# gunrock/graphblast

Hardware: NVIDIA H100
Metric: MTEPS (higher is better)
Workload: dtype f32

## Files before the change

graphblast_b200/csrc/graphblas/backend/cuda/kernels/bfs_fused.cuh:

```cuda
#ifndef GRAPHBLAS_BACKEND_CUDA_KERNELS_BFS_FUSED_CUH_
#define GRAPHBLAS_BACKEND_CUDA_KERNELS_BFS_FUSED_CUH_

#include <cooperative_groups.h>

#include "graphblas/backend/cuda/kernels/common.cuh"

namespace graphblas {
namespace backend {

#ifndef GB_BFS_NT
#define GB_BFS_NT     512
#endif
#ifndef GB_BFS_MINB
#define GB_BFS_MINB   2
#endif
#ifndef GB_BFS_PUSH_NT
#define GB_BFS_PUSH_NT   768
#endif
#ifndef GB_BFS_PUSH_MINB
#define GB_BFS_PUSH_MINB 2
#endif
#ifndef GB_BFS_BATCH
#define GB_BFS_BATCH  4
#endif
#ifndef GB_BFS_WALK_STEP
#define GB_BFS_WALK_STEP 4
#endif
#ifndef GB_BFS_WALK_WARP
#define GB_BFS_WALK_WARP 32
#endif
#ifndef GB_BFS_WALK_INLINE
#define GB_BFS_WALK_INLINE 64
#endif
#define GB_BFS_HEAVY  2048
#define GB_BFS_HEAVY_CAP 4096
#define GB_BFS_CHUNK  1024

struct BfsFusedArgs {
  const Index* push_ptr;   const Index* push_ind;
  const Index* pull_ptr;   const Index* pull_ind;
  const Index* pull_probe;
  const unsigned int* pull_empty;
  const unsigned int* push_empty;
  int   trace;
  unsigned long long* prof_bytes;
  Index n;
  Index source;
  int   max_levels;
  float switchpoint;
  int   mode;
  float*        levels;
  unsigned char* level8;
  unsigned int* visited[2];
  unsigned int* frontier;
  unsigned int* next;
  unsigned long long* counters;
  Index*        heavy;
  Index*        walk;
  int*          walk_count;
  Index*        walk_chunks;
};

#define GB_BFS_TIMED_LEVELS 16

enum BfsCell {
  GB_BFS_CELL_FOUND = 0,
  GB_BFS_CELL_HEAVY = GB_BFS_CELL_FOUND + 3,
  GB_BFS_CELL_LEVELS = GB_BFS_CELL_HEAVY + 3,
  GB_BFS_CELL_INSPECTED,
  GB_BFS_CELL_PULL_LEVELS,
  GB_BFS_CELL_PUSHED_VERTICES,
  GB_BFS_CELL_PUSHED_EDGES,
  GB_BFS_CELL_FOUND_PUSHING,
  GB_BFS_CELL_LEVEL_CLOCK,
  GB_BFS_CELL_START_CLOCK = GB_BFS_CELL_LEVEL_CLOCK + GB_BFS_TIMED_LEVELS,
  GB_BFS_CELL_END_PASS_CLOCK,
  GB_BFS_CELL_LAST_LEVEL_CLOCK,
  GB_BFS_CELL_WALK_CLAIM = 35,
  GB_BFS_CELL_LISTED = GB_BFS_CELL_WALK_CLAIM + 3,
  GB_BFS_CELL_SCAN_CLOCK = 44,
  GB_BFS_CELL_WALKED = GB_BFS_CELL_SCAN_CLOCK + GB_BFS_TIMED_LEVELS,
  GB_BFS_CELL_LISTED_CHUNKS = GB_BFS_CELL_WALKED + GB_BFS_TIMED_LEVELS,
  GB_BFS_NCOUNTERS = 128
};
static_assert(GB_BFS_CELL_LISTED_CHUNKS + GB_BFS_TIMED_LEVELS <= GB_BFS_NCOUNTERS,
              "the per-level cells of the last timed level are past the counters");

__device__ __forceinline__ unsigned long long* bfsLevelCell(unsigned long long* cells,
                                                            int first, int level) {
  return cells + first + level % 3;
}
__device__ __forceinline__ void bfsZeroNextCell(unsigned long long* cells, int first,
                                                int level) {
  cells[first + (level + 1) % 3] = 0ull;
}

__device__ __forceinline__ unsigned long long bfsClockNs() {
  unsigned long long t;
  asm volatile("mov.u64 %0, %globaltimer;" : "=l"(t));
  return t;
}

template <typename V>
__device__ __forceinline__ bool bfsClaim(unsigned int* visited, V vtx) {
  const unsigned int bit = 1u << (vtx & 31);
  unsigned int* word = visited + (vtx >> 5);
  if (*reinterpret_cast<volatile unsigned int*>(word) & bit) return false;
  return (atomicOr(word, bit) & bit) == 0;
}

__device__ __forceinline__ void bfsSetLevel(const BfsFusedArgs& a, Index row, int lv) {
  if (lv < 255) {
    a.level8[row] = static_cast<unsigned char>(lv);
  } else {
    a.level8[row] = 255;
    a.levels[row] = static_cast<float>(lv);
  }
}

__device__ __forceinline__ Index bfsClaimChunk(unsigned long long* cell, int lane) {
  unsigned long long c = 0ull;
  if (lane == 0) c = atomicAdd(cell, 1ull);
  return static_cast<Index>(__shfl_sync(GB_FULL_MASK, c, 0));
}

__device__ __forceinline__ unsigned int* bfsVis(const BfsFusedArgs& a, int vsel) {
  return vsel ? a.visited[1] : a.visited[0];
}
__device__ __forceinline__ unsigned int* bfsVisOther(const BfsFusedArgs& a, int vsel) {
  return vsel ? a.visited[0] : a.visited[1];
}
__device__ __forceinline__ unsigned int* bfsF(const BfsFusedArgs& a, int fsel) {
  return fsel ? a.next : a.frontier;
}
__device__ __forceinline__ unsigned int* bfsN(const BfsFusedArgs& a, int fsel) {
  return fsel ? a.frontier : a.next;
}

__device__ __forceinline__ unsigned int bfsIsolated(const BfsFusedArgs& a, Index w) {
  return a.pull_empty[w] & (a.push_empty != NULL ? a.push_empty[w] : 0xffffffffu);
}

__device__ __forceinline__ bool bfsWalkRows(const BfsFusedArgs& a, int vsel, Index row,
                                            bool active, int lane, int& inspected) {
  Index k = 0, end = 0;
  if (active) {
    k = __ldg(a.pull_ptr + row);
    end = __ldg(a.pull_ptr + row + 1);
  }
  const Index stop = (end - k > GB_BFS_WALK_WARP + GB_BFS_WALK_STEP)
                     ? k + GB_BFS_WALK_STEP : end;
  bool found = false;
  while (k < stop && !found) {
    Index col[GB_BFS_WALK_STEP];
    unsigned int wv[GB_BFS_WALK_STEP];
#pragma unroll
    for (int u = 0; u < GB_BFS_WALK_STEP; ++u)
      col[u] = (k + u < stop) ? __ldg(a.pull_ind + k + u) : static_cast<Index>(-1);
#pragma unroll
    for (int u = 0; u < GB_BFS_WALK_STEP; ++u)
      wv[u] = (col[u] >= 0) ? bfsVis(a, vsel)[col[u] >> 5] : 0u;
#pragma unroll
    for (int u = 0; u < GB_BFS_WALK_STEP; ++u) {
      if (found || col[u] < 0) continue;
      ++inspected;
      found = (wv[u] >> (col[u] & 31)) & 1u;
    }
    k += GB_BFS_WALK_STEP;
  }
  unsigned int longs = __ballot_sync(GB_FULL_MASK, !found && k < end);
  while (longs != 0u) {
    const int src = __ffs(longs) - 1;
    longs &= longs - 1u;
    const Index lend = __shfl_sync(GB_FULL_MASK, end, src);
    bool hit = false;
    for (Index lk = __shfl_sync(GB_FULL_MASK, k, src); lk < lend && !hit; lk += 32) {
      bool v = false;
      if (lk + lane < lend) {
        const Index col = __ldg(a.pull_ind + lk + lane);
        v = (bfsVis(a, vsel)[col >> 5] >> (col & 31)) & 1u;
      }
      const unsigned int b = __ballot_sync(GB_FULL_MASK, v);
      hit = (b != 0u);
      if (lane == 0)
        inspected += hit ? __ffs(b) : (lend - lk < 32 ? lend - lk : 32);
    }
    if (lane == src) found = hit;
  }
  return found;
}

template <int NT, int MINB, bool PULL>
__global__ void __launch_bounds__(NT, MINB)
bfsFusedKernel(BfsFusedArgs a) {
  namespace cg = cooperative_groups;
  cg::grid_group grid = cg::this_grid();
  __shared__ int s_red[NT/32];
  __shared__ unsigned int s_found[PULL ? NT/32 : 1][PULL ? 32 : 1];

  const Index n = a.n;
  const Index nwords = (n + 31) >> 5;
  const int lane = threadIdx.x & 31;
  const Index gtid = blockIdx.x*NT + threadIdx.x;
  const Index gthreads = gridDim.x*NT;
  const Index gwarp = gtid >> 5;
  const Index gwarps = gthreads >> 5;
  const Index nchunks = (nwords + 31) >> 5;

  if (gtid == 0) a.counters[GB_BFS_CELL_START_CLOCK] = bfsClockNs();
  if (gtid == 0) a.level8[a.source] = 1;
  for (Index w = gtid; w < nwords; w += gthreads) {
    const unsigned int seed = (w == (a.source >> 5)) ? (1u << (a.source & 31)) : 0u;
    a.visited[0][w] = seed | bfsIsolated(a, w);
    a.visited[1][w] = 0u; a.frontier[w] = seed; a.next[w] = 0u;
  }
  if (gtid <= GB_BFS_CELL_FOUND_PUSHING) a.counters[gtid] = 0ull;
  if (gtid >= GB_BFS_CELL_WALK_CLAIM && gtid < GB_BFS_CELL_LISTED + 3) a.counters[gtid] = 0ull;
  if (gtid >= GB_BFS_CELL_WALKED && gtid < GB_BFS_CELL_WALKED + GB_BFS_TIMED_LEVELS)
    a.counters[gtid] = 0ull;
  grid.sync();
  if (gtid == 0) a.counters[GB_BFS_CELL_LEVEL_CLOCK] = bfsClockNs() << 1;

  int vsel = 0;
  int fsel = 0;
  unsigned int fcount = 1u;
  bool dense = PULL && (a.mode == 2);
  float prev_ratio = 0.f;
  int inspected = 0;
  int pushed_vertices = 0;
  unsigned int pushed_edges = 0u;
  int pull_levels = 0;
  int level = 1;

  for (; level <= a.max_levels && fcount > 0u; ++level) {
    if (PULL && a.mode == 0) {
      const float ratio = static_cast<float>(fcount)/static_cast<float>(n);
      if (!dense) {
        if (ratio > a.switchpoint && ratio > prev_ratio) dense = true; else prev_ratio = ratio;
      } else {
        if (ratio <= a.switchpoint && ratio < prev_ratio) dense = false; else prev_ratio = ratio;
      }
    }
    unsigned long long* const count_cell = bfsLevelCell(a.counters, GB_BFS_CELL_FOUND, level);
    unsigned long long* const heavy_cell = bfsLevelCell(a.counters, GB_BFS_CELL_HEAVY, level);
    if (gtid == 0) {
      bfsZeroNextCell(a.counters, GB_BFS_CELL_FOUND, level);
      bfsZeroNextCell(a.counters, GB_BFS_CELL_HEAVY, level);
      bfsZeroNextCell(a.counters, GB_BFS_CELL_WALK_CLAIM, level);
      bfsZeroNextCell(a.counters, GB_BFS_CELL_LISTED, level);
    }
    int found_here = 0;

    if (!dense) {
      for (Index w0 = gwarp*32; w0 < nwords; w0 += gwarps*32) {
        const Index mine = w0 + lane;
        unsigned int my_bits = (mine < nwords) ? bfsF(a, fsel)[mine] : 0u;
        if (my_bits != 0u) bfsF(a, fsel)[mine] = 0u;
        unsigned int pending = __ballot_sync(GB_FULL_MASK, my_bits != 0u);
        while (pending != 0u) {
          const int src_lane = __ffs(pending) - 1;
          pending &= pending - 1u;
          unsigned int bits = __shfl_sync(GB_FULL_MASK, my_bits, src_lane);
          const Index w = w0 + src_lane;
          while (bits != 0u) {
            const int b = __ffs(bits) - 1;
            bits &= bits - 1u;
            const Index u = w*32 + b;
            const Index beg = __ldg(a.push_ptr + u);
            const Index deg = __ldg(a.push_ptr + u + 1) - beg;
            if (lane == 0) { ++pushed_vertices; pushed_edges += deg; }
            if (deg > GB_BFS_HEAVY) {
              unsigned long long slot = 0ull;
              if (lane == 0) slot = atomicAdd(heavy_cell, 1ull);
              slot = __shfl_sync(GB_FULL_MASK, slot, 0);
              if (slot < GB_BFS_HEAVY_CAP) {
                if (lane == 0) a.heavy[slot] = u;
                continue;
              }
            }
            for (Index k = lane; k < deg; k += 32) {
              const Index nbr = __ldg(a.push_ind + beg + k);
              if (bfsClaim(bfsVis(a, vsel), nbr)) {
                bfsSetLevel(a, nbr, level + 1);
                atomicOr(bfsN(a, fsel) + (nbr >> 5), 1u << (nbr & 31));
                ++found_here;
              }
            }
          }
        }
      }
      grid.sync();
      const unsigned long long listed =
          *reinterpret_cast<volatile unsigned long long*>(heavy_cell);
      const int nheavy = (listed > GB_BFS_HEAVY_CAP) ? GB_BFS_HEAVY_CAP
                                                     : static_cast<int>(listed);
      if (nheavy > 0) {
        for (int h = 0; h < nheavy; ++h) {
          const Index u = a.heavy[h];
          const Index beg = __ldg(a.push_ptr + u);
          const Index deg = __ldg(a.push_ptr + u + 1) - beg;
          for (Index k = gtid; k < deg; k += gthreads) {
            const Index nbr = __ldg(a.push_ind + beg + k);
            if (bfsClaim(bfsVis(a, vsel), nbr)) {
              bfsSetLevel(a, nbr, level + 1);
              atomicOr(bfsN(a, fsel) + (nbr >> 5), 1u << (nbr & 31));
              ++found_here;
            }
          }
        }
      }
    } else if (PULL) {
      ++pull_levels;
      unsigned long long* const walk_cell =
          bfsLevelCell(a.counters, GB_BFS_CELL_WALK_CLAIM, level);
      unsigned long long* const list_cell = bfsLevelCell(a.counters, GB_BFS_CELL_LISTED, level);
      Index c = gwarp;
      unsigned int next_vis = (c < nchunks && c*32 + lane < nwords)
                              ? bfsVis(a, vsel)[c*32 + lane] : 0xffffffffu;
      while (c < nchunks) {
        const Index word = c*32 + lane;
        const unsigned int my_vis = next_vis;
        const Index c_next = c + gwarps;
        next_vis = (c_next < nchunks && c_next*32 + lane < nwords)
                   ? bfsVis(a, vsel)[c_next*32 + lane] : 0xffffffffu;
        Index* const walk = a.walk + c*GB_BFS_CHUNK;
        int nwalk = 0;
        unsigned int my_out = 0u;
        unsigned int open = __ballot_sync(GB_FULL_MASK, my_vis != 0xffffffffu);
        unsigned int my_open = ~my_vis;
        if (word == nwords - 1 && (n & 31) != 0) my_open &= (1u << (n & 31)) - 1u;
        const int nopen = __popc(my_open);
        int first = nopen;
#pragma unroll
        for (int off = 1; off < 32; off <<= 1) {
          const int t = __shfl_up_sync(GB_FULL_MASK, first, off);
          if (lane >= off) first += t;
        }
        const int total = __shfl_sync(GB_FULL_MASK, first, 31);
        first -= nopen;
        const int word_batches = (__popc(open) + GB_BFS_BATCH - 1)/GB_BFS_BATCH;
        const int row_batches = (total + 32*GB_BFS_BATCH - 1)/(32*GB_BFS_BATCH);
        if (2*row_batches < word_batches) {
          open = 0u;
          unsigned int* const found_bits = s_found[threadIdx.x >> 5];
          found_bits[lane] = 0u;
          __syncwarp();
          for (int r0 = 0; r0 < total; r0 += 32*GB_BFS_BATCH) {
            int local[GB_BFS_BATCH];
            Index f[GB_BFS_BATCH];
#pragma unroll
            for (int j = 0; j < GB_BFS_BATCH; ++j) {
              const int r = r0 + 32*j + lane;
              int wl = 0, base = 0;
#pragma unroll
              for (int step = 16; step > 0; step >>= 1) {
                const int fs = __shfl_sync(GB_FULL_MASK, first, wl + step);
                if (fs <= r) { wl += step; base = fs; }
              }
              unsigned int m = __shfl_sync(GB_FULL_MASK, my_open, wl);
              int k = r - base, b = 0;
#pragma unroll
              for (int width = 16; width > 0; width >>= 1) {
                const int lo = __popc(m & ((1u << width) - 1u));
                if (k >= lo) { k -= lo; b += width; m >>= width; }
              }
              local[j] = wl*32 + b;
              f[j] = (r < total) ? ldStream32(a.pull_probe + c*GB_BFS_CHUNK + local[j])
                                 : static_cast<Index>(-1);
            }
            unsigned int pword[GB_BFS_BATCH];
#pragma unroll
            for (int j = 0; j < GB_BFS_BATCH; ++j)
              pword[j] = (f[j] != static_cast<Index>(-1))
                         ? bfsVis(a, vsel)[(f[j] & 0x7fffffff) >> 5] : 0u;
#pragma unroll
            for (int j = 0; j < GB_BFS_BATCH; ++j) {
              if (r0 + 32*j >= total) break;
              const bool found = (pword[j] >> (f[j] & 31)) & 1u;
              inspected += (f[j] != static_cast<Index>(-1)) ? 1 : 0;
              const bool walk_row = f[j] >= 0 && !found;
              const Index row = c*GB_BFS_CHUNK + local[j];
              const unsigned int walkers = __ballot_sync(GB_FULL_MASK, walk_row);
              if (walk_row) walk[nwalk + __popc(walkers & ((1u << lane) - 1u))] = row;
              nwalk += __popc(walkers);
              if (found) {
                atomicOr(found_bits + (local[j] >> 5), 1u << (local[j] & 31));
                bfsSetLevel(a, row, level + 1);
                ++found_here;
              }
            }
          }
          __syncwarp();
          my_out = found_bits[lane];
        }
        while (open != 0u) {
          const unsigned int batch = open;
          Index f[GB_BFS_BATCH];
#pragma unroll
          for (int j = 0; j < GB_BFS_BATCH; ++j) {
            const int wl = __ffs(open) - 1;
            open &= open - 1u;
            f[j] = static_cast<Index>(-1);
            if (wl >= 0) {
              const unsigned int m = __shfl_sync(GB_FULL_MASK, my_vis, wl);
              const Index row = c*GB_BFS_CHUNK + wl*32 + lane;
              if (row < n && !((m >> lane) & 1u)) f[j] = ldStream32(a.pull_probe + row);
            }
          }
          unsigned int pword[GB_BFS_BATCH];
#pragma unroll
          for (int j = 0; j < GB_BFS_BATCH; ++j)
            pword[j] = (f[j] != static_cast<Index>(-1))
                       ? bfsVis(a, vsel)[(f[j] & 0x7fffffff) >> 5] : 0u;
          unsigned int hit = 0u, more = 0u;
#pragma unroll
          for (int j = 0; j < GB_BFS_BATCH; ++j) {
            const bool found = (pword[j] >> (f[j] & 31)) & 1u;
            inspected += (f[j] != static_cast<Index>(-1)) ? 1 : 0;
            hit |= static_cast<unsigned int>(found) << j;
            more |= static_cast<unsigned int>(f[j] >= 0 && !found) << j;
          }
          unsigned int rest = batch;
#pragma unroll
          for (int j = 0; j < GB_BFS_BATCH && rest != 0u; ++j) {
            const int wl = __ffs(rest) - 1;
            rest &= rest - 1u;
            const Index row = c*GB_BFS_CHUNK + wl*32 + lane;
            const bool found = (hit >> j) & 1u, walk_row = (more >> j) & 1u;
            const unsigned int walkers = __ballot_sync(GB_FULL_MASK, walk_row);
            if (walk_row) walk[nwalk + __popc(walkers & ((1u << lane) - 1u))] = row;
            nwalk += __popc(walkers);
            const unsigned int out = __ballot_sync(GB_FULL_MASK, found);
            if (found) { bfsSetLevel(a, row, level + 1); ++found_here; }
            if (lane == wl) my_out = out;
          }
        }
        if (nwalk > 0 && nwalk <= GB_BFS_WALK_INLINE) {
          unsigned int* const found_bits = s_found[threadIdx.x >> 5];
          found_bits[lane] = my_out;
          __syncwarp();
          for (int i0 = 0; i0 < nwalk; i0 += 32) {
            const bool active = i0 + lane < nwalk;
            const Index row = active ? walk[i0 + lane] : 0;
            if (bfsWalkRows(a, vsel, row, active, lane, inspected)) {
              const int local = row & (GB_BFS_CHUNK - 1);
              atomicOr(found_bits + (local >> 5), 1u << (local & 31));
              bfsSetLevel(a, row, level + 1);
              ++found_here;
            }
          }
          __syncwarp();
          my_out = found_bits[lane];
        }
        if (word < nwords) {
          bfsN(a, fsel)[word] = my_out;
          bfsVisOther(a, vsel)[word] = my_vis | my_out;
          bfsF(a, fsel)[word] = 0u;
        }
        if (lane == 0 && nwalk > 0) {
          if (nwalk > GB_BFS_WALK_INLINE) {
            a.walk_count[c] = nwalk;
            a.walk_chunks[atomicAdd(list_cell, 1ull)] = c;
          }
          if (a.trace && level < GB_BFS_TIMED_LEVELS)
            atomicAdd(a.counters + GB_BFS_CELL_WALKED + level,
                      static_cast<unsigned long long>(nwalk));
        }
        c = c_next;
      }
      grid.sync();
      const Index nlisted = static_cast<Index>(
          *reinterpret_cast<volatile unsigned long long*>(list_cell));
      if (gtid == 0 && level < GB_BFS_TIMED_LEVELS) {
        a.counters[GB_BFS_CELL_SCAN_CLOCK + level] = bfsClockNs();
        if (a.trace)
          a.counters[GB_BFS_CELL_LISTED_CHUNKS + level] = static_cast<unsigned long long>(nlisted);
      }
      for (Index i = gwarp; i < nlisted; ) {
        const Index i_next = gwarps + bfsClaimChunk(walk_cell, lane);
        const Index c = a.walk_chunks[i];
        const int nwalk = a.walk_count[c];
        for (int i0 = 0; i0 < nwalk; i0 += 32) {
          const bool active = i0 + lane < nwalk;
          const Index row = active ? a.walk[c*GB_BFS_CHUNK + i0 + lane] : 0;
          if (bfsWalkRows(a, vsel, row, active, lane, inspected)) {
            const unsigned int bit = 1u << (row & 31);
            atomicOr(bfsN(a, fsel) + (row >> 5), bit);
            atomicOr(bfsVisOther(a, vsel) + (row >> 5), bit);
            bfsSetLevel(a, row, level + 1);
            ++found_here;
          }
        }
        i = i_next;
      }
    }
    const int block_found = blockSum<NT>(found_here, s_red);
    if (threadIdx.x == 0 && block_found) {
      atomicAdd(count_cell, static_cast<unsigned long long>(block_found));
      if (!dense)
        atomicAdd(a.counters + GB_BFS_CELL_FOUND_PUSHING,
                  static_cast<unsigned long long>(block_found));
    }
    grid.sync();
    if (gtid == 0 && level < GB_BFS_TIMED_LEVELS)
      a.counters[GB_BFS_CELL_LEVEL_CLOCK + level] = (bfsClockNs() << 1) | (dense ? 1ull : 0ull);
    fcount = static_cast<unsigned int>(
        *reinterpret_cast<volatile unsigned long long*>(count_cell));
    if (dense) vsel ^= 1;
    fsel ^= 1;
  }
  if (gtid == 0) a.counters[GB_BFS_CELL_LAST_LEVEL_CLOCK] = bfsClockNs();
  const unsigned int* const cut_rows = (fcount > 0u) ? bfsF(a, fsel) : NULL;
  const bool lines = (reinterpret_cast<uintptr_t>(a.levels) & 15u) == 0u;
  const Index nblocks = (nwords + 15) >> 4;
  if (PULL) {
    auto load_block = [&](Index blk, unsigned int& reached, unsigned int (&b)[4]) {
      reached = 0u;
#pragma unroll
      for (int j = 0; j < 4; ++j) b[j] = 0u;
      if (blk >= nblocks) return;
      const Index w = blk*16 + (lane & 15);
      if (lane < 16 && w < nwords) {
        reached = bfsVis(a, vsel)[w] & ~bfsIsolated(a, w);
        if (cut_rows != NULL) reached &= ~cut_rows[w];
        if (w == (a.source >> 5)) reached |= 1u << (a.source & 31);
      }
#pragma unroll
      for (int j = 0; j < 4; ++j) {
        const Index row = blk*512 + 128*j + 4*lane;
        if (lines && row + 4 <= n) b[j] = *reinterpret_cast<const unsigned int*>(a.level8 + row);
      }
    };
    unsigned int next_reached, next_b[4];
    load_block(gwarp, next_reached, next_b);
    for (Index blk = gwarp; blk < nblocks; blk += gwarps) {
      const Index r0 = blk*512;
      const unsigned int reached = next_reached;
      unsigned int lb[4];
#pragma unroll
      for (int j = 0; j < 4; ++j) lb[j] = next_b[j];
      load_block(blk + gwarps, next_reached, next_b);
#pragma unroll
      for (int j = 0; j < 4; ++j) {
        const unsigned int bits =
            (__shfl_sync(GB_FULL_MASK, reached, 4*j + (lane >> 3)) >> (4*(lane & 7))) & 0xfu;
        const Index row = r0 + 128*j + 4*lane;
        if (row >= n) continue;
        if (lines && row + 4 <= n) {
          const unsigned int b = lb[j];
          float f[4];
          bool escape = false;
#pragma unroll
          for (int k = 0; k < 4; ++k) {
            const unsigned int byte = (b >> (8*k)) & 0xffu;
            const bool r = (bits >> k) & 1u;
            escape |= r && byte == 255u;
            f[k] = r ? static_cast<float>(byte) : 0.f;
          }
          if (!escape) {
            __stcs(reinterpret_cast<float4*>(a.levels + row), make_float4(f[0], f[1], f[2], f[3]));
            continue;
          }
        }
        for (int k = 0; k < 4 && row + k < n; ++k) {
          if (!((bits >> k) & 1u)) {
            a.levels[row + k] = 0.f;
          } else {
            const unsigned int byte = a.level8[row + k];
            if (byte != 255u) a.levels[row + k] = static_cast<float>(byte);
          }
        }
      }
    }
  } else {
    for (Index blk = gwarp; blk < nblocks; blk += gwarps) {
      const Index r0 = blk*512;
      const Index w = blk*16 + (lane & 15);
      unsigned int reached = 0u;
      if (lane < 16 && w < nwords) {
        reached = bfsVis(a, vsel)[w] & ~bfsIsolated(a, w);
        if (cut_rows != NULL) reached &= ~cut_rows[w];
        if (w == (a.source >> 5)) reached |= 1u << (a.source & 31);
      }
#pragma unroll
      for (int j = 0; j < 4; ++j) {
        const unsigned int bits =
            (__shfl_sync(GB_FULL_MASK, reached, 4*j + (lane >> 3)) >> (4*(lane & 7))) & 0xfu;
        const Index row = r0 + 128*j + 4*lane;
        if (row >= n) continue;
        if (lines && row + 4 <= n) {
          const unsigned int b = *reinterpret_cast<const unsigned int*>(a.level8 + row);
          float f[4];
          bool escape = false;
#pragma unroll
          for (int k = 0; k < 4; ++k) {
            const unsigned int byte = (b >> (8*k)) & 0xffu;
            const bool r = (bits >> k) & 1u;
            escape |= r && byte == 255u;
            f[k] = r ? static_cast<float>(byte) : 0.f;
          }
          if (!escape) {
            __stcs(reinterpret_cast<float4*>(a.levels + row), make_float4(f[0], f[1], f[2], f[3]));
            continue;
          }
        }
        for (int k = 0; k < 4 && row + k < n; ++k) {
          if (!((bits >> k) & 1u)) {
            a.levels[row + k] = 0.f;
          } else {
            const unsigned int byte = a.level8[row + k];
            if (byte != 255u) a.levels[row + k] = static_cast<float>(byte);
          }
        }
      }
    }
  }
  if (a.trace) {
    grid.sync();
    if (gtid == 0) a.counters[GB_BFS_CELL_END_PASS_CLOCK] = bfsClockNs();
  }
  const int block_insp = blockSum<NT>(inspected, s_red);
  const int block_pv = blockSum<NT>(pushed_vertices, s_red);
  if (threadIdx.x == 0) {
    if (block_insp)
      atomicAdd(a.counters + GB_BFS_CELL_INSPECTED, static_cast<unsigned long long>(block_insp));
    if (block_pv)
      atomicAdd(a.counters + GB_BFS_CELL_PUSHED_VERTICES,
                static_cast<unsigned long long>(block_pv));
  }
  if (pushed_edges)
    atomicAdd(a.counters + GB_BFS_CELL_PUSHED_EDGES,
              static_cast<unsigned long long>(pushed_edges));
  if (gtid == 0) {
    a.counters[GB_BFS_CELL_LEVELS] = static_cast<unsigned long long>(level - 1);
    a.counters[GB_BFS_CELL_PULL_LEVELS] = static_cast<unsigned long long>(pull_levels);
  }
  if (a.prof_bytes != NULL) {
    if (pushed_edges) atomicAdd(a.prof_bytes, 8ull*pushed_edges);
    if (threadIdx.x == 0) {
      unsigned long long bytes = 4ull*static_cast<unsigned long long>(block_insp) +
                                 12ull*static_cast<unsigned long long>(block_pv);
      if (blockIdx.x == 0)
        bytes += static_cast<unsigned long long>(pull_levels)*
                     (12ull*static_cast<unsigned long long>(n) + 4ull) +
                 8ull*(*reinterpret_cast<volatile unsigned long long*>(
                           a.counters + GB_BFS_CELL_FOUND_PUSHING));
      if (bytes) atomicAdd(a.prof_bytes, bytes);
    }
  }
}

}
}

#endif
```

graphblast_b200/csrc/graphblas/backend/cuda/bfs_fused.hpp:

```cpp
#ifndef GRAPHBLAS_BACKEND_CUDA_BFS_FUSED_HPP_
#define GRAPHBLAS_BACKEND_CUDA_BFS_FUSED_HPP_

#include "graphblas/backend/cuda/kernels/bfs_fused.cuh"

namespace graphblas {
namespace backend {

inline bool bfsFusedApplies(Descriptor* desc) {
  Desc_value mask_mode, outp, inp0, inp1;
  if (desc->get(GrB_MASK, &mask_mode) != GrB_SUCCESS) return false;
  desc->get(GrB_OUTP, &outp); desc->get(GrB_INP0, &inp0); desc->get(GrB_INP1, &inp1);
  return desc->struconly() && desc->opreuse() && desc->earlyexit() && desc->fusedmask() &&
         mask_mode == GrB_DEFAULT && outp == GrB_DEFAULT && inp0 == GrB_DEFAULT &&
         inp1 == GrB_DEFAULT && !desc->debug() && desc->timing_ != 1;
}

inline bool bfsTrace() {
  static const bool on = getEnv("GB200_BFS_TRACE", 0) != 0;
  return on;
}

struct BfsScratchLayout {
  size_t visited[2], frontier, next, counters, heavy, walk, walk_count, walk_chunks,
         level8, bytes;
};

inline BfsScratchLayout bfsScratchLayout(Index n) {
  const size_t nwords = (static_cast<size_t>(n) + 31)/32;
  const size_t nchunks = (nwords + 31)/32;
  BfsScratchLayout l;
  size_t at = 0;
  auto place = [&at](size_t bytes) {
    const size_t off = at;
    at += (bytes + 255)/256*256;
    return off;
  };
  l.visited[0]  = place(nwords*sizeof(unsigned int));
  l.visited[1]  = place(nwords*sizeof(unsigned int));
  l.frontier    = place(nwords*sizeof(unsigned int));
  l.next        = place(nwords*sizeof(unsigned int));
  l.counters    = place(GB_BFS_NCOUNTERS*sizeof(unsigned long long));
  l.heavy       = place(GB_BFS_HEAVY_CAP*sizeof(Index));
  l.walk        = place(nchunks*GB_BFS_CHUNK*sizeof(Index));
  l.walk_count  = place(nchunks*sizeof(int));
  l.walk_chunks = place(nchunks*sizeof(Index));
  l.level8      = place(static_cast<size_t>(n));
  l.bytes = at;
  return l;
}

inline void bfsFusedStats(Descriptor* desc, Index n, unsigned long long out[6]) {
  static_assert(GB_BFS_CELL_FOUND_PUSHING == GB_BFS_CELL_LEVELS + 5,
                "the six result cells are not consecutive");
  for (int i = 0; i < 6; ++i) out[i] = 0ull;
  const BfsScratchLayout l = bfsScratchLayout(n);
  const size_t cells = l.counters + GB_BFS_CELL_LEVELS*sizeof(unsigned long long);
  if (desc->scratchSize(GB_SCRATCH_BFS) < cells + 6*sizeof(unsigned long long)) return;
  unsigned char* base = reinterpret_cast<unsigned char*>(desc->scratch(GB_SCRATCH_BFS, 0));
  CUDA_CALL(cudaMemcpyAsync(out, base + cells, 6*sizeof(unsigned long long),
      cudaMemcpyDeviceToHost, gbStream()));
  runtime().sync();
}

template <typename a>
Info bfsFused(Vector<float>* v, const Matrix<a>* A, Index s, Descriptor* desc, int* depth) {
  SparseMatrix<a>* S = const_cast<SparseMatrix<a>*>(&A->sparse_);
  const Index n = S->nrows_;
  if (n != S->ncols_) return GrB_DIMENSION_MISMATCH;
  if (S->d_csrRowPtr_ == NULL || S->d_cscColPtr_ == NULL) return GrB_UNINITIALIZED_OBJECT;
  cudaStream_t stream = gbStream();
  CHECK(v->setStorage(GrB_DENSE));
  CHECK(v->dense_.allocateGpu());

  const int fw = 1;
  const Index* probe = pullMaxDegreeNeighbours(S, fw, S->d_cscColPtr_, S->d_cscRowInd_, n);

  const BfsScratchLayout l = bfsScratchLayout(n);
  unsigned char* base =
      reinterpret_cast<unsigned char*>(desc->scratch(GB_SCRATCH_BFS, l.bytes));
  BfsFusedArgs args;
  args.push_ptr = S->d_csrRowPtr_;  args.push_ind = S->d_csrColInd_;
  args.pull_ptr = S->d_cscColPtr_;  args.pull_ind = S->d_cscRowInd_;
  args.pull_probe = probe;
  args.pull_empty = pullEmptyRowBits(probe, n);
  args.push_empty = S->sameStructure() ? NULL : pullEmptyRowBits(
      pullFirstNeighbours(S, 0, S->d_csrRowPtr_, S->d_csrColInd_, n), n);
  args.n = n;
  args.source = s;
  args.max_levels = desc->max_niter_;
  args.switchpoint = desc->switchpoint();
  Desc_value mode;
  CHECK(desc->get(GrB_MXVMODE, &mode));
  args.mode = (mode == GrB_PUSHONLY) ? 1 : (mode == GrB_PULLONLY ? 2 : 0);
  args.levels = v->dense_.d_val_;
  args.visited[0]  = reinterpret_cast<unsigned int*>(base + l.visited[0]);
  args.visited[1]  = reinterpret_cast<unsigned int*>(base + l.visited[1]);
  args.frontier    = reinterpret_cast<unsigned int*>(base + l.frontier);
  args.next        = reinterpret_cast<unsigned int*>(base + l.next);
  args.counters    = reinterpret_cast<unsigned long long*>(base + l.counters);
  args.heavy       = reinterpret_cast<Index*>(base + l.heavy);
  args.walk        = reinterpret_cast<Index*>(base + l.walk);
  args.walk_count  = reinterpret_cast<int*>(base + l.walk_count);
  args.walk_chunks = reinterpret_cast<Index*>(base + l.walk_chunks);
  args.level8      = base + l.level8;

  args.trace = bfsTrace();
  args.prof_bytes = NULL;
  if (profiler().enabled) {
    profiler().ensureCells();
    args.prof_bytes = profiler().d_cells + GB_PROF_PULL_BOOL;
  }

  const bool push_only = (args.mode == 1);
  void (*kernel)(BfsFusedArgs) =
      push_only ? bfsFusedKernel<GB_BFS_PUSH_NT, GB_BFS_PUSH_MINB, false>
                : bfsFusedKernel<GB_BFS_NT, GB_BFS_MINB, true>;
  const int nt = push_only ? GB_BFS_PUSH_NT : GB_BFS_NT;
  const int grid = push_only
      ? cooperativeGrid<bfsFusedKernel<GB_BFS_PUSH_NT, GB_BFS_PUSH_MINB, false>,
                        GB_BFS_PUSH_NT>()
      : cooperativeGrid<bfsFusedKernel<GB_BFS_NT, GB_BFS_MINB, true>, GB_BFS_NT>();
  if (grid < 1) return GrB_PANIC;
  void* params[] = { &args };
  profiler().begin(GB_PROF_PULL_BOOL, stream);
  CUDA_CALL(cudaLaunchCooperativeKernel(reinterpret_cast<void*>(kernel),
      dim3(grid), dim3(nt), params, 0, stream));
  GB_KERNEL_CHECK();
  profiler().end(GB_PROF_PULL_BOOL, stream, 0.0);
  v->dense_.touched();
  if (args.trace) {
    unsigned long long cells[GB_BFS_NCOUNTERS];
    CUDA_CALL(cudaMemcpyAsync(cells, args.counters, sizeof(cells), cudaMemcpyDeviceToHost,
        stream));
    runtime().sync();
    const unsigned long long* const clock = cells + GB_BFS_CELL_LEVEL_CLOCK;
    const int levels = static_cast<int>(
        cells[GB_BFS_CELL_LEVELS] < GB_BFS_TIMED_LEVELS - 1 ? cells[GB_BFS_CELL_LEVELS]
                                                            : GB_BFS_TIMED_LEVELS - 1);
    fprintf(stderr, "bfs trace: set-up %.1fus",
            1e-3*static_cast<double>((clock[0] >> 1) - cells[GB_BFS_CELL_START_CLOCK]));
    for (int l = 1; l <= levels; ++l) {
      const unsigned long long start = clock[l - 1] >> 1, end = clock[l] >> 1;
      const unsigned long long scan = cells[GB_BFS_CELL_SCAN_CLOCK + l];
      if (clock[l] & 1ull)
        fprintf(stderr, " L%d pull %.1fus (scan %.1f walk %.1f, %llu walked, %llu listed)",
                l, 1e-3*static_cast<double>(end - start),
                1e-3*static_cast<double>(scan - start),
                1e-3*static_cast<double>(end - scan), cells[GB_BFS_CELL_WALKED + l],
                cells[GB_BFS_CELL_LISTED_CHUNKS + l]);
      else
        fprintf(stderr, " L%d push %.1fus", l, 1e-3*static_cast<double>(end - start));
    }
    fprintf(stderr, " end-pass %.1fus\n",
            1e-3*static_cast<double>(cells[GB_BFS_CELL_END_PASS_CLOCK] -
                                     cells[GB_BFS_CELL_LAST_LEVEL_CLOCK]));
  }
  if (depth != NULL) {
    const unsigned long long levels = runtime().fetch(args.counters + GB_BFS_CELL_LEVELS);
    *depth = static_cast<int>(levels);
    desc->lastmxv_ = GrB_PULLONLY;
  }
  return GrB_SUCCESS;
}

}
}

#endif
```

Baseline: 2.432 million.

## Add dense-chunk path loading pull probes as 128-bit vectors per group

When many words in a chunk are open, a new path processes 128-row groups with each lane loading four consecutive probe entries through one 128-bit streaming load. The next group's load is software-pipelined against processing of the current one. Walk-list slots are computed with a warp prefix scan, and output bits are rebuilt with shuffles. This replaces per-word scalar probe loads in dense frontiers, at the cost of extra shuffle and scan work and a more complex boundary path.

New measurement: 2.485 million, median of 6. 1.02x the previous value.

```diff
diff --git a/graphblast_b200/csrc/graphblas/backend/cuda/kernels/bfs_fused.cuh b/graphblast_b200/csrc/graphblas/backend/cuda/kernels/bfs_fused.cuh
--- a/graphblast_b200/csrc/graphblas/backend/cuda/kernels/bfs_fused.cuh
+++ b/graphblast_b200/csrc/graphblas/backend/cuda/kernels/bfs_fused.cuh
@@ -22,6 +22,9 @@
 #endif
 #ifndef GB_BFS_BATCH
 #define GB_BFS_BATCH  4
+#endif
+#ifndef GB_BFS_DENSE_WORDS
+#define GB_BFS_DENSE_WORDS 16
 #endif
 #ifndef GB_BFS_WALK_STEP
 #define GB_BFS_WALK_STEP 4
@@ -393,6 +396,76 @@
           __syncwarp();
           my_out = found_bits[lane];
         }
+        if (__popc(open) > GB_BFS_DENSE_WORDS) {
+          open = 0u;
+          unsigned int groups = __ballot_sync(GB_FULL_MASK, my_open != 0u);
+          groups |= groups >> 1;
+          groups = (groups | (groups >> 2)) & 0x11111111u;
+          int4 fn = make_int4(-1, -1, -1, -1);
+          int gn = -1;
+          do {
+            const int4 fc = fn;
+            const int gc = gn;
+            gn = (groups != 0u) ? (__ffs(groups) - 1) >> 2 : -1;
+            groups &= groups - 1u;
+            {
+              const unsigned int bits = (__shfl_sync(GB_FULL_MASK, my_open, 4*gn + (lane >> 3))
+                                         >> (4*(lane & 7))) & 0xfu;
+              const Index row0 = c*GB_BFS_CHUNK + 128*gn + 4*lane;
+              fn = make_int4(-1, -1, -1, -1);
+              if (gn >= 0 && bits != 0u) {
+                if (row0 + 4 <= n + 1) fn = ldStream128(a.pull_probe + row0);
+                else {
+                  if (bits & 1u) fn.x = ldStream32(a.pull_probe + row0);
+                  if (bits & 2u) fn.y = ldStream32(a.pull_probe + row0 + 1);
+                  if (bits & 4u) fn.z = ldStream32(a.pull_probe + row0 + 2);
+                }
+                if (!(bits & 1u)) fn.x = -1;
+                if (!(bits & 2u)) fn.y = -1;
+                if (!(bits & 4u)) fn.z = -1;
+                if (!(bits & 8u)) fn.w = -1;
+              }
+            }
+            if (gc < 0) continue;
+            const Index f[4] = {fc.x, fc.y, fc.z, fc.w};
+            unsigned int pword[4];
+#pragma unroll
+            for (int k = 0; k < 4; ++k)
+              pword[k] = (f[k] != static_cast<Index>(-1))
+                         ? bfsVis(a, vsel)[(f[k] & 0x7fffffff) >> 5] : 0u;
+            unsigned int hit = 0u, more = 0u;
+#pragma unroll
+            for (int k = 0; k < 4; ++k) {
+              const bool found = (pword[k] >> (f[k] & 31)) & 1u;
+              inspected += (f[k] != static_cast<Index>(-1)) ? 1 : 0;
+              hit |= static_cast<unsigned int>(found) << k;
+              more |= static_cast<unsigned int>(f[k] >= 0 && !found) << k;
+            }
+            const int nmore = __popc(more);
+            int slot = nmore;
+#pragma unroll
+            for (int off = 1; off < 32; off <<= 1) {
+              const int t = __shfl_up_sync(GB_FULL_MASK, slot, off);
+              if (lane >= off) slot += t;
+            }
+            const int gwalk = __shfl_sync(GB_FULL_MASK, slot, 31);
+            slot += nwalk - nmore;
+            nwalk += gwalk;
+            const Index row0 = c*GB_BFS_CHUNK + 128*gc + 4*lane;
+#pragma unroll
+            for (int k = 0; k < 4; ++k) {
+              if ((more >> k) & 1u) walk[slot++] = row0 + k;
+              if ((hit >> k) & 1u) bfsSetLevel(a, row0 + k, level + 1);
+            }
+            found_here += __popc(hit);
+            unsigned int out = hit << (4*(lane & 7));
+            out |= __shfl_xor_sync(GB_FULL_MASK, out, 1);
+            out |= __shfl_xor_sync(GB_FULL_MASK, out, 2);
+            out |= __shfl_xor_sync(GB_FULL_MASK, out, 4);
+            out = __shfl_sync(GB_FULL_MASK, out, 8*(lane & 3));
+            if ((lane >> 2) == gc) my_out = out;
+          } while (gn >= 0);
+        }
         while (open != 0u) {
           const unsigned int batch = open;
           Index f[GB_BFS_BATCH];
```

## Keep an explicit frontier list for sparse push levels in fused BFS

Applied to the files above, without the earlier changes.

Push levels now append newly claimed vertices to a compacted, double-buffered frontier list using warp ballot and one atomic per warp. The next push level walks that list instead of scanning the whole frontier bitmap, and tiny frontiers get an edge-balanced path where each warp load-balances across the few vertices' edges. This targets the O(n/32) bitmap scan on sparse levels, at the cost of extra atomics and stores during claiming, plus a fallback to the bitmap scan when the list overflows. fsel is now derived from the level parity.

Measured after the change: 2.457 million before, 2.482 million after, median of 6. About the same (+1.0%).

```diff
diff --git a/graphblast_b200/csrc/graphblas/backend/cuda/bfs_fused.hpp b/graphblast_b200/csrc/graphblas/backend/cuda/bfs_fused.hpp
--- a/graphblast_b200/csrc/graphblas/backend/cuda/bfs_fused.hpp
+++ b/graphblast_b200/csrc/graphblas/backend/cuda/bfs_fused.hpp
@@ -21,8 +21,8 @@
 }
 
 struct BfsScratchLayout {
-  size_t visited[2], frontier, next, counters, heavy, walk, walk_count, walk_chunks,
-         level8, bytes;
+  size_t visited[2], frontier, next, counters, heavy, flist, walk, walk_count,
+         walk_chunks, level8, bytes;
 };
 
 inline BfsScratchLayout bfsScratchLayout(Index n) {
@@ -41,6 +41,7 @@
   l.next        = place(nwords*sizeof(unsigned int));
   l.counters    = place(GB_BFS_NCOUNTERS*sizeof(unsigned long long));
   l.heavy       = place(GB_BFS_HEAVY_CAP*sizeof(Index));
+  l.flist       = place(2*GB_BFS_FLIST_CAP*sizeof(Index));
   l.walk        = place(nchunks*GB_BFS_CHUNK*sizeof(Index));
   l.walk_count  = place(nchunks*sizeof(int));
   l.walk_chunks = place(nchunks*sizeof(Index));
@@ -99,6 +100,7 @@
   args.next        = reinterpret_cast<unsigned int*>(base + l.next);
   args.counters    = reinterpret_cast<unsigned long long*>(base + l.counters);
   args.heavy       = reinterpret_cast<Index*>(base + l.heavy);
+  args.flist       = reinterpret_cast<Index*>(base + l.flist);
   args.walk        = reinterpret_cast<Index*>(base + l.walk);
   args.walk_count  = reinterpret_cast<int*>(base + l.walk_count);
   args.walk_chunks = reinterpret_cast<Index*>(base + l.walk_chunks);
diff --git a/graphblast_b200/csrc/graphblas/backend/cuda/kernels/bfs_fused.cuh b/graphblast_b200/csrc/graphblas/backend/cuda/kernels/bfs_fused.cuh
--- a/graphblast_b200/csrc/graphblas/backend/cuda/kernels/bfs_fused.cuh
+++ b/graphblast_b200/csrc/graphblas/backend/cuda/kernels/bfs_fused.cuh
@@ -35,6 +35,8 @@
 #define GB_BFS_HEAVY  2048
 #define GB_BFS_HEAVY_CAP 4096
 #define GB_BFS_CHUNK  1024
+#define GB_BFS_FLIST_CAP 65536
+#define GB_BFS_FLIST_SHORT 32
 
 struct BfsFusedArgs {
   const Index* push_ptr;   const Index* push_ind;
@@ -56,6 +58,7 @@
   unsigned int* next;
   unsigned long long* counters;
   Index*        heavy;
+  Index*        flist;
   Index*        walk;
   int*          walk_count;
   Index*        walk_chunks;
@@ -66,7 +69,8 @@
 enum BfsCell {
   GB_BFS_CELL_FOUND = 0,
   GB_BFS_CELL_HEAVY = GB_BFS_CELL_FOUND + 3,
-  GB_BFS_CELL_LEVELS = GB_BFS_CELL_HEAVY + 3,
+  GB_BFS_CELL_FLIST = GB_BFS_CELL_HEAVY + 3,
+  GB_BFS_CELL_LEVELS = GB_BFS_CELL_FLIST + 3,
   GB_BFS_CELL_INSPECTED,
   GB_BFS_CELL_PULL_LEVELS,
   GB_BFS_CELL_PUSHED_VERTICES,
@@ -83,6 +87,8 @@
   GB_BFS_CELL_LISTED_CHUNKS = GB_BFS_CELL_WALKED + GB_BFS_TIMED_LEVELS,
   GB_BFS_NCOUNTERS = 128
 };
+static_assert(GB_BFS_CELL_LAST_LEVEL_CLOCK < GB_BFS_CELL_WALK_CLAIM,
+              "the clocks overlap the pull levels' cells");
 static_assert(GB_BFS_CELL_LISTED_CHUNKS + GB_BFS_TIMED_LEVELS <= GB_BFS_NCOUNTERS,
               "the per-level cells of the last timed level are past the counters");
 
@@ -93,6 +99,12 @@
 __device__ __forceinline__ void bfsZeroNextCell(unsigned long long* cells, int first,
                                                 int level) {
   cells[first + (level + 1) % 3] = 0ull;
+}
+
+__device__ __forceinline__ Index bfsGridCtas() {
+  unsigned int c;
+  asm volatile("mov.u32 %0, %%nctaid.x;" : "=r"(c));
+  return static_cast<Index>(c);
 }
 
 __device__ __forceinline__ unsigned long long bfsClockNs() {
@@ -107,6 +119,25 @@
   unsigned int* word = visited + (vtx >> 5);
   if (*reinterpret_cast<volatile unsigned int*>(word) & bit) return false;
   return (atomicOr(word, bit) & bit) == 0;
+}
+
+__device__ __forceinline__ Index* bfsList(const BfsFusedArgs& a, int level) {
+  return a.flist + (level & 1)*GB_BFS_FLIST_CAP;
+}
+
+__device__ __forceinline__ void bfsAppend(const BfsFusedArgs& a, int level, Index vtx,
+                                          bool won, int lane, bool& append) {
+  const unsigned int winners = __ballot_sync(GB_FULL_MASK, won);
+  if (winners == 0u) return;
+  unsigned int base = 0u;
+  if (lane == 0)
+    base = static_cast<unsigned int>(atomicAdd(
+        bfsLevelCell(a.counters, GB_BFS_CELL_FLIST, level),
+        static_cast<unsigned long long>(__popc(winners))));
+  base = __shfl_sync(GB_FULL_MASK, base, 0);
+  const unsigned int slot = base + __popc(winners & ((1u << lane) - 1u));
+  if (won && slot < GB_BFS_FLIST_CAP) bfsList(a, level)[slot] = vtx;
+  if (base + __popc(winners) > GB_BFS_FLIST_CAP) append = false;
 }
 
 __device__ __forceinline__ void bfsSetLevel(const BfsFusedArgs& a, Index row, int lv) {
@@ -208,13 +239,14 @@
   const Index nchunks = (nwords + 31) >> 5;
 
   if (gtid == 0) a.counters[GB_BFS_CELL_START_CLOCK] = bfsClockNs();
-  if (gtid == 0) a.level8[a.source] = 1;
+  if (gtid == 0) { a.level8[a.source] = 1; bfsList(a, 0)[0] = a.source; }
   for (Index w = gtid; w < nwords; w += gthreads) {
     const unsigned int seed = (w == (a.source >> 5)) ? (1u << (a.source & 31)) : 0u;
     a.visited[0][w] = seed | bfsIsolated(a, w);
     a.visited[1][w] = 0u; a.frontier[w] = seed; a.next[w] = 0u;
   }
-  if (gtid <= GB_BFS_CELL_FOUND_PUSHING) a.counters[gtid] = 0ull;
+  if (gtid <= GB_BFS_CELL_FOUND_PUSHING)
+    a.counters[gtid] = (gtid == GB_BFS_CELL_FLIST) ? 1ull : 0ull;
   if (gtid >= GB_BFS_CELL_WALK_CLAIM && gtid < GB_BFS_CELL_LISTED + 3) a.counters[gtid] = 0ull;
   if (gtid >= GB_BFS_CELL_WALKED && gtid < GB_BFS_CELL_WALKED + GB_BFS_TIMED_LEVELS)
     a.counters[gtid] = 0ull;
@@ -222,7 +254,6 @@
   if (gtid == 0) a.counters[GB_BFS_CELL_LEVEL_CLOCK] = bfsClockNs() << 1;
 
   int vsel = 0;
-  int fsel = 0;
   unsigned int fcount = 1u;
   bool dense = PULL && (a.mode == 2);
   float prev_ratio = 0.f;
@@ -241,71 +272,122 @@
         if (ratio <= a.switchpoint && ratio < prev_ratio) dense = false; else prev_ratio = ratio;
       }
     }
+    const int fsel = (level - 1) & 1;
     unsigned long long* const count_cell = bfsLevelCell(a.counters, GB_BFS_CELL_FOUND, level);
-    unsigned long long* const heavy_cell = bfsLevelCell(a.counters, GB_BFS_CELL_HEAVY, level);
     if (gtid == 0) {
       bfsZeroNextCell(a.counters, GB_BFS_CELL_FOUND, level);
       bfsZeroNextCell(a.counters, GB_BFS_CELL_HEAVY, level);
+      bfsZeroNextCell(a.counters, GB_BFS_CELL_FLIST, level);
       bfsZeroNextCell(a.counters, GB_BFS_CELL_WALK_CLAIM, level);
       bfsZeroNextCell(a.counters, GB_BFS_CELL_LISTED, level);
     }
     int found_here = 0;
 
     if (!dense) {
-      for (Index w0 = gwarp*32; w0 < nwords; w0 += gwarps*32) {
-        const Index mine = w0 + lane;
-        unsigned int my_bits = (mine < nwords) ? bfsF(a, fsel)[mine] : 0u;
-        if (my_bits != 0u) bfsF(a, fsel)[mine] = 0u;
-        unsigned int pending = __ballot_sync(GB_FULL_MASK, my_bits != 0u);
-        while (pending != 0u) {
-          const int src_lane = __ffs(pending) - 1;
-          pending &= pending - 1u;
-          unsigned int bits = __shfl_sync(GB_FULL_MASK, my_bits, src_lane);
-          const Index w = w0 + src_lane;
-          while (bits != 0u) {
-            const int b = __ffs(bits) - 1;
-            bits &= bits - 1u;
-            const Index u = w*32 + b;
-            const Index beg = __ldg(a.push_ptr + u);
-            const Index deg = __ldg(a.push_ptr + u + 1) - beg;
-            if (lane == 0) { ++pushed_vertices; pushed_edges += deg; }
-            if (deg > GB_BFS_HEAVY) {
-              unsigned long long slot = 0ull;
-              if (lane == 0) slot = atomicAdd(heavy_cell, 1ull);
-              slot = __shfl_sync(GB_FULL_MASK, slot, 0);
-              if (slot < GB_BFS_HEAVY_CAP) {
-                if (lane == 0) a.heavy[slot] = u;
-                continue;
+      bool append = PULL;
+      auto claim = [&](Index nbr) {
+        if (!bfsClaim(bfsVis(a, vsel), nbr)) return false;
+        bfsSetLevel(a, nbr, level + 1);
+        atomicOr(bfsN(a, fsel) + (nbr >> 5), 1u << (nbr & 31));
+        ++found_here;
+        return true;
+      };
+      auto claim_list = [&](Index nbr) {
+        const bool won = nbr >= 0 && claim(nbr);
+        if (append) bfsAppend(a, level, nbr, won, lane, append);
+      };
+      auto push_vertex = [&](Index u) {
+        const Index beg = __ldg(a.push_ptr + u);
+        const Index deg = __ldg(a.push_ptr + u + 1) - beg;
+        if (lane == 0) { ++pushed_vertices; pushed_edges += deg; }
+        if (deg > GB_BFS_HEAVY) {
+          unsigned long long slot = 0ull;
+          if (lane == 0) slot = atomicAdd(bfsLevelCell(a.counters, GB_BFS_CELL_HEAVY, level), 1ull);
+          slot = __shfl_sync(GB_FULL_MASK, slot, 0);
+          if (slot < GB_BFS_HEAVY_CAP) {
+            if (lane == 0) a.heavy[slot] = u;
+            return;
+          }
+        }
+        if (append) {
+          for (Index k0 = 0; k0 < deg; k0 += 32)
+            claim_list(k0 + lane < deg ? __ldg(a.push_ind + beg + k0 + lane) : -1);
+        } else {
+          for (Index k = lane; k < deg; k += 32) claim(__ldg(a.push_ind + beg + k));
+        }
+      };
+      const unsigned long long nlist = *reinterpret_cast<volatile unsigned long long*>(
+          bfsLevelCell(a.counters, GB_BFS_CELL_FLIST, level - 1));
+      const bool listed_frontier = PULL && nlist == fcount && nlist <= GB_BFS_FLIST_CAP;
+      if (listed_frontier && fcount <= GB_BFS_FLIST_SHORT) {
+        Index beg = 0, deg = 0;
+        if (lane < static_cast<int>(fcount)) {
+          const Index u = bfsList(a, level - 1)[lane];
+          beg = __ldg(a.push_ptr + u);
+          deg = __ldg(a.push_ptr + u + 1) - beg;
+          if (gwarp == 0) bfsF(a, fsel)[u >> 5] = 0u;
+        }
+        Index first = deg;
+#pragma unroll
+        for (int off = 1; off < 32; off <<= 1) {
+          const Index t = __shfl_up_sync(GB_FULL_MASK, first, off);
+          if (lane >= off) first += t;
+        }
+        const Index total = __shfl_sync(GB_FULL_MASK, first, 31);
+        first -= deg;
+        if (gtid == 0) { pushed_vertices += fcount; pushed_edges += total; }
+        append = total <= GB_BFS_FLIST_CAP;
+        for (Index e0 = gwarp*32; e0 < total; e0 += bfsGridCtas()*NT) {
+          const Index e = e0 + lane;
+          int j = 0;
+#pragma unroll
+          for (int step = 16; step > 0; step >>= 1)
+            if (__shfl_sync(GB_FULL_MASK, first, j + step) <= e) j += step;
+          const Index jbeg = __shfl_sync(GB_FULL_MASK, beg, j);
+          const Index jfirst = __shfl_sync(GB_FULL_MASK, first, j);
+          claim_list(e < total ? __ldg(a.push_ind + jbeg + e - jfirst) : -1);
+        }
+      } else {
+        if (listed_frontier) {
+          for (Index i = gwarp; i < static_cast<Index>(fcount); i += bfsGridCtas()*(NT/32)) {
+            const Index u = bfsList(a, level - 1)[i];
+            if (lane == 0) bfsF(a, fsel)[u >> 5] = 0u;
+            push_vertex(u);
+          }
+        } else {
+          for (Index w0 = gwarp*32; w0 < nwords; w0 += bfsGridCtas()*NT) {
+            const Index mine = w0 + lane;
+            unsigned int my_bits = (mine < nwords) ? bfsF(a, fsel)[mine] : 0u;
+            if (my_bits != 0u) bfsF(a, fsel)[mine] = 0u;
+            unsigned int pending = __ballot_sync(GB_FULL_MASK, my_bits != 0u);
+            while (pending != 0u) {
+              const int src_lane = __ffs(pending) - 1;
+              pending &= pending - 1u;
+              unsigned int bits = __shfl_sync(GB_FULL_MASK, my_bits, src_lane);
+              const Index w = w0 + src_lane;
+              while (bits != 0u) {
+                const int b = __ffs(bits) - 1;
+                bits &= bits - 1u;
+                push_vertex(w*32 + b);
               }
             }
-            for (Index k = lane; k < deg; k += 32) {
-              const Index nbr = __ldg(a.push_ind + beg + k);
-              if (bfsClaim(bfsVis(a, vsel), nbr)) {
-                bfsSetLevel(a, nbr, level + 1);
-                atomicOr(bfsN(a, fsel) + (nbr >> 5), 1u << (nbr & 31));
-                ++found_here;
-              }
-            }
-          }
-        }
-      }
-      grid.sync();
-      const unsigned long long listed =
-          *reinterpret_cast<volatile unsigned long long*>(heavy_cell);
-      const int nheavy = (listed > GB_BFS_HEAVY_CAP) ? GB_BFS_HEAVY_CAP
-                                                     : static_cast<int>(listed);
-      if (nheavy > 0) {
+          }
+        }
+        grid.sync();
+        const unsigned long long listed =
+            *reinterpret_cast<volatile unsigned long long*>(
+                bfsLevelCell(a.counters, GB_BFS_CELL_HEAVY, level));
+        const int nheavy = (listed > GB_BFS_HEAVY_CAP) ? GB_BFS_HEAVY_CAP
+                                                       : static_cast<int>(listed);
         for (int h = 0; h < nheavy; ++h) {
           const Index u = a.heavy[h];
           const Index beg = __ldg(a.push_ptr + u);
           const Index deg = __ldg(a.push_ptr + u + 1) - beg;
-          for (Index k = gtid; k < deg; k += gthreads) {
-            const Index nbr = __ldg(a.push_ind + beg + k);
-            if (bfsClaim(bfsVis(a, vsel), nbr)) {
-              bfsSetLevel(a, nbr, level + 1);
-              atomicOr(bfsN(a, fsel) + (nbr >> 5), 1u << (nbr & 31));
-              ++found_here;
-            }
+          if (append) {
+            for (Index k0 = gwarp*32; k0 < deg; k0 += bfsGridCtas()*NT)
+              claim_list(k0 + lane < deg ? __ldg(a.push_ind + beg + k0 + lane) : -1);
+          } else {
+            for (Index k = gtid; k < deg; k += bfsGridCtas()*NT) claim(__ldg(a.push_ind + beg + k));
           }
         }
       }
@@ -507,10 +589,9 @@
     fcount = static_cast<unsigned int>(
         *reinterpret_cast<volatile unsigned long long*>(count_cell));
     if (dense) vsel ^= 1;
-    fsel ^= 1;
   }
   if (gtid == 0) a.counters[GB_BFS_CELL_LAST_LEVEL_CLOCK] = bfsClockNs();
-  const unsigned int* const cut_rows = (fcount > 0u) ? bfsF(a, fsel) : NULL;
+  const unsigned int* const cut_rows = (fcount > 0u) ? bfsF(a, (level - 1) & 1) : NULL;
   const bool lines = (reinterpret_cast<uintptr_t>(a.levels) & 15u) == 0u;
   const Index nblocks = (nwords + 15) >> 4;
   if (PULL) {
```
